# interstellar/zkvm

Measured on AMD Instinct MI355X. Metric: ZkVM tx verifications/sec (batch), higher is better.
Workload: dtype u32 limb pairs of radix-2^51 (v_mad_u64_u32)

## Files before the change

zkvm_amd/csrc/kernels.hpp:

```cpp
#pragma once
#include "curve.hpp"
#include "quad.hpp"
#include "sc_dev.hpp"

namespace zk {

constexpr uint32_t ENTRY_NEG = 1u << 31;
constexpr uint32_t ENTRY_DYN = 1u << 30;
constexpr uint32_t ENTRY_IDX = (1u << 30) - 1;
constexpr int NIELS_WORDS = 32;
constexpr int EXT_WORDS = 40;
constexpr int REDUCE_CHUNK = 64;
#ifndef ZK_REDUCE_CHUNK_BIG
#define ZK_REDUCE_CHUNK_BIG 16
#endif
constexpr int REDUCE_CHUNK_BIG = ZK_REDUCE_CHUNK_BIG;
constexpr int TABLE_WORDS = 24;
constexpr int TABLE_STRIDE = 32;

struct JobDesc {
  const uint32_t* dyn_scalars;
  const uint64_t* dyn_offsets;
  uint64_t n_dyn;
  const uint32_t* st_scalars;
  const uint32_t* st_index;
  const uint64_t* st_offsets;
  uint64_t n_static;
  uint32_t n_msm;
  int w;
  int n_windows;
  uint32_t n_buckets;
};


__device__ __forceinline__ void load_niels(ge_niels& q, const uint32_t* row) {
  const uint4* r4 = reinterpret_cast<const uint4*>(row);
  uint32_t w[32];
#pragma unroll
  for (int i = 0; i < 8; ++i) {
    uint4 v = r4[i];
    w[4 * i] = v.x; w[4 * i + 1] = v.y; w[4 * i + 2] = v.z; w[4 * i + 3] = v.w;
  }
#pragma unroll
  for (int i = 0; i < 10; ++i) { q.ypx.v[i] = w[i]; q.ymx.v[i] = w[10 + i]; q.xy2d.v[i] = w[20 + i]; }
}

__device__ __forceinline__ void store_niels(uint32_t* row, const ge_niels& q, uint32_t valid) {
  uint32_t w[32];
#pragma unroll
  for (int i = 0; i < 10; ++i) { w[i] = q.ypx.v[i]; w[10 + i] = q.ymx.v[i]; w[20 + i] = q.xy2d.v[i]; }
  w[30] = valid; w[31] = 0;
  uint4* r4 = reinterpret_cast<uint4*>(row);
#pragma unroll
  for (int i = 0; i < 8; ++i) r4[i] = make_uint4(w[4 * i], w[4 * i + 1], w[4 * i + 2], w[4 * i + 3]);
}

__device__ __forceinline__ void load_ext(ge& p, const uint32_t* row) {
  const uint4* r4 = reinterpret_cast<const uint4*>(row);
  uint32_t w[40];
#pragma unroll
  for (int i = 0; i < 10; ++i) {
    uint4 v = r4[i];
    w[4 * i] = v.x; w[4 * i + 1] = v.y; w[4 * i + 2] = v.z; w[4 * i + 3] = v.w;
  }
#pragma unroll
  for (int i = 0; i < 10; ++i) { p.X.v[i] = w[i]; p.Y.v[i] = w[10 + i]; p.Z.v[i] = w[20 + i]; p.T.v[i] = w[30 + i]; }
}

__device__ __forceinline__ void store_ext(uint32_t* row, const ge& p) {
  uint32_t w[40];
#pragma unroll
  for (int i = 0; i < 10; ++i) { w[i] = p.X.v[i]; w[10 + i] = p.Y.v[i]; w[20 + i] = p.Z.v[i]; w[30 + i] = p.T.v[i]; }
  uint4* r4 = reinterpret_cast<uint4*>(row);
#pragma unroll
  for (int i = 0; i < 10; ++i) r4[i] = make_uint4(w[4 * i], w[4 * i + 1], w[4 * i + 2], w[4 * i + 3]);
}

__device__ __forceinline__ void load_table_row(ge_niels& q, const uint32_t* row) {
  const uint4* r4 = reinterpret_cast<const uint4*>(row);
  uint32_t w[24];
#pragma unroll
  for (int i = 0; i < 6; ++i) {
    uint4 v = r4[i];
    w[4 * i] = v.x; w[4 * i + 1] = v.y; w[4 * i + 2] = v.z; w[4 * i + 3] = v.w;
  }
  fe_from_words(q.ypx, w);
  fe_from_words(q.ymx, w + 8);
  fe_from_words(q.xy2d, w + 16);
}

__device__ __forceinline__ void store_table_row(uint32_t* row, const ge_niels& q) {
  uint32_t w[24];
  fe_to_words(w, q.ypx);
  fe_to_words(w + 8, q.ymx);
  fe_to_words(w + 16, q.xy2d);
  uint4* r4 = reinterpret_cast<uint4*>(row);
#pragma unroll
  for (int i = 0; i < 6; ++i) r4[i] = make_uint4(w[4 * i], w[4 * i + 1], w[4 * i + 2], w[4 * i + 3]);
}

__device__ __forceinline__ uint32_t find_row(const uint64_t* __restrict__ offsets, uint32_t n_msm, uint64_t g) {
  uint32_t lo = 0, hi = n_msm;
  while (hi - lo > 1) {
    uint32_t mid = (lo + hi) >> 1;
    if (offsets[mid] <= g) lo = mid; else hi = mid;
  }
  return lo;
}

__global__ void __launch_bounds__(256)
k_decompress(const uint32_t* __restrict__ pts, uint32_t* __restrict__ rows, uint64_t n,
             const uint64_t* __restrict__ offsets, uint32_t n_msm, uint32_t* __restrict__ msm_fail,
             unsigned long long* __restrict__ bad_index, uint8_t* __restrict__ ok_out) {
  uint64_t i = (uint64_t)blockIdx.x * blockDim.x + threadIdx.x;
  if (i >= n) return;
  const uint4* p4 = reinterpret_cast<const uint4*>(pts + 8 * i);
  uint4 a = p4[0], b = p4[1];
  uint32_t w[8] = {a.x, a.y, a.z, a.w, b.x, b.y, b.z, b.w};
  fe x, y;
  bool ok = ristretto_decode_affine(x, y, w);
  ge_niels q;
  niels_from_affine(q, x, y);
  if (!ok) niels_identity(q);
  if (rows) store_niels(rows + NIELS_WORDS * i, q, ok ? 1u : 0u);
  if (ok_out) ok_out[i] = ok ? 1 : 0;
  if (!ok) {
    if (bad_index) atomicMin(bad_index, (unsigned long long)i);
    if (msm_fail) {
      uint32_t m = (n_msm > 1 && offsets) ? find_row(offsets, n_msm, i) : 0;
      atomicOr(&msm_fail[m], 1u);
    }
  }
}

struct DecodeRoutes {
  uint64_t n[4] = {0, 0, 0, 0};
  void note(bool split, uint64_t points) {
    n[split ? 2 : 0] += 1;
    n[split ? 3 : 1] += points;
  }
};

constexpr int DEC_WORDS = 64;

struct DecFront { fe s, u1, u2, v, w, w7; bool pre_ok; };
__device__ __forceinline__ void dec_front(DecFront& d, const uint32_t* __restrict__ pts, uint64_t i) {
  const uint4* p4 = reinterpret_cast<const uint4*>(pts + 8 * i);
  uint4 a = p4[0], b = p4[1];
  uint32_t w[8] = {a.x, a.y, a.z, a.w, b.x, b.y, b.z, b.w};
  fe ss, u2_sqr, t;
  fe_from_words(d.s, w);
  uint32_t chk[8];
  fe_to_words(chk, d.s);
  bool canonical = true;
#pragma unroll
  for (int k = 0; k < 8; ++k) canonical &= (chk[k] == w[k]);
  d.pre_ok = canonical && !(w[0] & 1);
  fe_sq(ss, d.s);
  fe_sub(d.u1, fe_one(), ss);
  fe_add(d.u2, fe_one(), ss);
  fe_carry(d.u1);
  fe_carry(d.u2);
  fe_sq(u2_sqr, d.u2);
  fe_sq(t, d.u1);
  fe_mul(t, t, fe_D());
  fe_add(t, t, u2_sqr);
  fe_sub_c(d.v, fe_zero(), t);
  fe_mul(d.w, d.v, u2_sqr);
  fe w2, w3;
  fe_sq(w2, d.w);
  fe_mul(w3, w2, d.w);
  fe_sq(d.w7, w3);
  fe_mul(d.w7, d.w7, d.w);
}

__global__ void __launch_bounds__(256)
k_decompress_pre(const uint32_t* __restrict__ pts, uint32_t* __restrict__ scratch, uint64_t n) {
  const uint64_t i = (uint64_t)blockIdx.x * blockDim.x + threadIdx.x;
  if (i >= n) return;
  DecFront d;
  dec_front(d, pts, i);
  uint32_t* col = scratch + (uint64_t)50 * n + i;
#pragma unroll
  for (int k = 0; k < 10; ++k) col[(uint64_t)k * n] = d.w7.v[k];
}

#ifndef ZK_POW_WAVES
#define ZK_POW_WAVES 3
#endif
__global__ void __launch_bounds__(256, ZK_POW_WAVES)
k_pow22523(uint32_t* __restrict__ scratch, uint64_t n) {
  const uint64_t i = (uint64_t)blockIdx.x * blockDim.x + threadIdx.x;
  if (i >= n) return;
  uint32_t* col = scratch + (uint64_t)50 * n + i;
  fe x, r;
#pragma unroll
  for (int k = 0; k < 10; ++k) x.v[k] = col[(uint64_t)k * n];
  fe_pow22523(r, x);
#pragma unroll
  for (int k = 0; k < 10; ++k) col[(uint64_t)k * n] = r.v[k];
}

__global__ void __launch_bounds__(256)
k_decompress_post(const uint32_t* __restrict__ pts, const uint32_t* __restrict__ scratch, uint32_t* __restrict__ rows, uint64_t n,
                  const uint64_t* __restrict__ offsets, uint32_t n_msm, uint32_t* __restrict__ msm_fail,
                  unsigned long long* __restrict__ bad_index) {
  const uint64_t i = (uint64_t)blockIdx.x * blockDim.x + threadIdx.x;
  if (i >= n) return;
  DecFront d;
  dec_front(d, pts, i);
  const fe s = d.s, u1 = d.u1, u2 = d.u2, v = d.v, w = d.w;
  const bool pre_ok = d.pre_ok;
  const uint32_t* col = scratch + (uint64_t)50 * n + i;
  fe pw;
#pragma unroll
  for (int k = 0; k < 10; ++k) pw.v[k] = col[(uint64_t)k * n];
  fe w3, r, t, check, r_prime, neg_r;
  fe_sq(t, w);
  fe_mul(w3, t, w);
  fe_mul(r, pw, w3);
  fe_sq(t, r);
  fe_mul(check, t, w);
  const fe one = fe_one();
  fe neg_one, neg_i;
  fe_neg(neg_one, one);
  fe_mul(neg_i, neg_one, fe_SQRT_M1());
  const bool correct_sign = fe_eq(check, one);
  const bool flipped_sign = fe_eq(check, neg_one);
  const bool flipped_sign_i = fe_eq(check, neg_i);
  fe_mul(r_prime, r, fe_SQRT_M1());
  fe_cmov(r, r_prime, flipped_sign | flipped_sign_i);
  fe_neg(neg_r, r);
  fe_cmov(r, neg_r, fe_is_negative(r));
  const bool was_square = correct_sign | flipped_sign;
  fe den_x, den_y, x, y, nx;
  fe_mul(den_x, r, u2);
  fe_mul(den_y, r, den_x);
  fe_mul(den_y, den_y, v);
  fe_mul(x, s, den_x);
  fe_add(x, x, x);
  fe_carry(x);
  fe_neg(nx, x);
  fe_cmov(x, nx, fe_is_negative(x));
  fe_mul(y, u1, den_y);
  fe_mul(t, x, y);
  const bool ok = pre_ok & was_square & !fe_is_negative(t) & !fe_is_zero(y);
  ge_niels q;
  niels_from_affine(q, x, y);
  if (!ok) niels_identity(q);
  store_niels(rows + NIELS_WORDS * i, q, ok ? 1u : 0u);
  if (!ok) {
    if (bad_index) atomicMin(bad_index, (unsigned long long)i);
    if (msm_fail) {
      uint32_t m = (n_msm > 1 && offsets) ? find_row(offsets, n_msm, i) : 0;
      atomicOr(&msm_fail[m], 1u);
    }
  }
}

template <typename F>
__device__ __forceinline__ void for_each_digit(const uint32_t* __restrict__ sc, int w, int n_windows, F f) {
  uint32_t s[8];
  const uint4* s4 = reinterpret_cast<const uint4*>(sc);
  uint4 a = s4[0], b = s4[1];
  s[0] = a.x; s[1] = a.y; s[2] = a.z; s[3] = a.w; s[4] = b.x; s[5] = b.y; s[6] = b.z; s[7] = b.w;
  const uint32_t mask = (1u << w) - 1, half = 1u << (w - 1);
  uint32_t carry = 0;
  for (int t = 0; t < n_windows; ++t) {
    const int pos = t * w;
    uint32_t bits = 0;
    if (pos < 256) {
      const int idx = pos >> 5, sh = pos & 31;
      uint32_t lo = 0, hi = 0;
#pragma unroll
      for (int k = 0; k < 8; ++k) { lo = (k == idx) ? s[k] : lo; hi = (k == idx + 1) ? s[k] : hi; }
      uint64_t two = (uint64_t)lo | ((uint64_t)hi << 32);
      bits = (uint32_t)(two >> sh) & mask;
    }
    uint32_t v = bits + carry;
    int d;
    if (v > half) { d = (int)v - (int)(mask + 1); carry = 1; }
    else { d = (int)v; carry = 0; }
    if (d != 0) f(t, d);
  }
}

__device__ __forceinline__ void term_lookup(const JobDesc& j, uint64_t g, const uint32_t*& sc, uint32_t& m,
                                            uint32_t& entry) {
  if (g < j.n_dyn) {
    sc = j.dyn_scalars + 8 * g;
    m = (j.n_msm > 1) ? find_row(j.dyn_offsets, j.n_msm, g) : 0;
    entry = ENTRY_DYN | (uint32_t)g;
  } else {
    const uint64_t k = g - j.n_dyn;
    sc = j.st_scalars + 8 * k;
    m = (j.n_msm > 1) ? find_row(j.st_offsets, j.n_msm, k) : 0;
    entry = j.st_index ? j.st_index[k] : (uint32_t)(k - (j.n_msm > 1 ? j.st_offsets[m] : 0));
  }
}

__global__ void __launch_bounds__(256)
k_digits_count(JobDesc j, uint32_t* __restrict__ hist, uint32_t* __restrict__ status) {
  uint64_t g = (uint64_t)blockIdx.x * blockDim.x + threadIdx.x;
  if (g >= j.n_dyn + j.n_static) return;
  const uint32_t* sc; uint32_t m, entry;
  term_lookup(j, g, sc, m, entry);
  if (sc[7] >> 31) atomicOr(&status[0], 2u);
  const uint64_t base = (uint64_t)m * j.n_windows;
  for_each_digit(sc, j.w, j.n_windows, [&](int t, int d) {
    const uint32_t b = (uint32_t)(d < 0 ? -d : d) - 1;
    atomicAdd(&hist[(base + t) * j.n_buckets + b], 1u);
  });
}

__global__ void __launch_bounds__(256)
k_digits_scatter(JobDesc j, uint32_t* __restrict__ cursor, uint32_t* __restrict__ entries) {
  uint64_t g = (uint64_t)blockIdx.x * blockDim.x + threadIdx.x;
  if (g >= j.n_dyn + j.n_static) return;
  const uint32_t* sc; uint32_t m, entry;
  term_lookup(j, g, sc, m, entry);
  const uint64_t base = (uint64_t)m * j.n_windows;
  for_each_digit(sc, j.w, j.n_windows, [&](int t, int d) {
    const uint32_t b = (uint32_t)(d < 0 ? -d : d) - 1;
    const uint32_t pos = atomicAdd(&cursor[(base + t) * j.n_buckets + b], 1u);
    entries[pos] = entry | (d < 0 ? ENTRY_NEG : 0u);
  });
}

constexpr int SCAN_ITEMS = 8;
constexpr int SCAN_BLOCK = 256;
constexpr int SCAN_TILE = SCAN_ITEMS * SCAN_BLOCK;

__device__ __forceinline__ uint32_t block_exclusive_scan(uint32_t v, uint32_t& total) {
  __shared__ uint32_t wave_tot[SCAN_BLOCK / 64];
  const int lane = threadIdx.x & 63, wid = threadIdx.x >> 6;
  uint32_t x = v;
#pragma unroll
  for (int o = 1; o < 64; o <<= 1) {
    uint32_t y = __shfl_up(x, o);
    if (lane >= o) x += y;
  }
  if (lane == 63) wave_tot[wid] = x;
  __syncthreads();
  uint32_t base = 0, tot = 0;
#pragma unroll
  for (int k = 0; k < SCAN_BLOCK / 64; ++k) {
    uint32_t wt = wave_tot[k];
    if (k < wid) base += wt;
    tot += wt;
  }
  __syncthreads();
  total = tot;
  return base + x - v;
}

__global__ void __launch_bounds__(SCAN_BLOCK)
k_scan_reduce(const uint32_t* __restrict__ in, uint64_t n, uint32_t* __restrict__ block_sums) {
  const uint64_t base = (uint64_t)blockIdx.x * SCAN_TILE + (uint64_t)threadIdx.x * SCAN_ITEMS;
  uint32_t s = 0;
#pragma unroll
  for (int k = 0; k < SCAN_ITEMS; ++k) if (base + k < n) s += in[base + k];
  uint32_t total;
  (void)block_exclusive_scan(s, total);
  if (threadIdx.x == 0) block_sums[blockIdx.x] = total;
}

__global__ void __launch_bounds__(SCAN_BLOCK)
k_scan_blocksums(uint32_t* __restrict__ block_sums, uint32_t n_blocks) {
  uint32_t carry = 0;
  for (uint32_t start = 0; start < n_blocks; start += SCAN_BLOCK) {
    const uint32_t i = start + threadIdx.x;
    uint32_t v = i < n_blocks ? block_sums[i] : 0;
    uint32_t total;
    uint32_t ex = block_exclusive_scan(v, total);
    if (i < n_blocks) block_sums[i] = carry + ex;
    carry += total;
  }
}

__global__ void __launch_bounds__(SCAN_BLOCK)
k_scan_apply(uint32_t* __restrict__ data, uint64_t n, const uint32_t* __restrict__ block_sums) {
  const uint64_t base = (uint64_t)blockIdx.x * SCAN_TILE + (uint64_t)threadIdx.x * SCAN_ITEMS;
  uint32_t v[SCAN_ITEMS], s = 0;
#pragma unroll
  for (int k = 0; k < SCAN_ITEMS; ++k) { v[k] = (base + k < n) ? data[base + k] : 0; s += v[k]; }
  uint32_t total;
  uint32_t ex = block_exclusive_scan(s, total) + block_sums[blockIdx.x];
#pragma unroll
  for (int k = 0; k < SCAN_ITEMS; ++k) { if (base + k < n) data[base + k] = ex; ex += v[k]; }
}

// ... 487 lines not shown
  fe_add(h, b, a);
  fe_sub(f, d, c);
  fe_add(g, d, c);
  fe_cswap(f, g, negate);
  fe_mul(r.X, e, f);
  fe_mul(r.Y, g, h);
  fe_mul(r.Z, f, g);
  fe_mul(r.T, e, h);
}

constexpr int SMALL_TBL = 8;

__device__ __forceinline__ void store_cached(uint32_t* row, const ge& p) {
  ge c4;
  fe_add_c(c4.X, p.Y, p.X);
  fe_sub_c(c4.Y, p.Y, p.X);
  fe_add_c(c4.Z, p.Z, p.Z);
  fe_mul(c4.T, p.T, fe_D2());
  store_ext(row, c4);
}

__global__ void __launch_bounds__(64)
k_small_tables(const uint32_t* __restrict__ dyn_scalars, const uint32_t* __restrict__ dyn_rows, uint64_t n,
               uint32_t* __restrict__ tbl , uint32_t* __restrict__ recoded ,
               uint32_t* __restrict__ status) {
  const uint64_t k = (uint64_t)blockIdx.x * 64 + threadIdx.x;
  if (k >= n) return;
  if (dyn_scalars) {
    const uint32_t* sc = dyn_scalars + 8 * k;
    if (sc[7] >> 31) atomicOr(&status[0], 2u);
    uint32_t carry = 0;
#pragma unroll
    for (int i = 0; i < 8; ++i) {
      const uint64_t v = (uint64_t)sc[i] + 0x88888888u + carry;
      recoded[8 * k + i] = (uint32_t)v;
      carry = (uint32_t)(v >> 32);
    }
  }
  ge_niels nq;
  load_niels(nq, dyn_rows + k * NIELS_WORDS);
  ge cur;
  ge_identity(cur);
  uint32_t* row = tbl + k * (SMALL_TBL * EXT_WORDS);
#pragma unroll 1
  for (int e = 0; e < SMALL_TBL; ++e) {
    ge_madd(cur, cur, nq, false);
    store_cached(row + e * EXT_WORDS, cur);
  }
}

__global__ void __launch_bounds__(256)
k_small_accumulate(const uint32_t* __restrict__ recoded, const uint64_t* __restrict__ dyn_offsets,
                   const uint32_t* __restrict__ tbl, uint32_t n_msm, uint32_t* __restrict__ window_sums,
                   uint32_t* __restrict__ window_nonempty) {
  extern __shared__ __attribute__((aligned(16))) uint32_t smem[];
  const uint32_t m = blockIdx.x;
  const int t = threadIdx.x & 63;
  const int part = threadIdx.x >> 6, parts = blockDim.x >> 6;
  const uint64_t k0 = dyn_offsets[m], k1 = dyn_offsets[m + 1];
  ge total;
  bool total_set = false;
#pragma unroll 1
  for (uint64_t k = k0 + part; k < k1; k += parts) {
    const uint32_t n4 = (recoded[8 * k + (t >> 3)] >> (4 * (t & 7))) & 15u;
    const int d = (t == 63 && n4 < 8u) ? (int)n4 + 8 : (int)n4 - 8;
    if (d != 0) {
      ge c4;
      load_ext(c4, tbl + (k * SMALL_TBL + (uint64_t)((d < 0 ? -d : d) - 1)) * EXT_WORDS);
      ge_cached c;
      c.YpX = c4.X; c.YmX = c4.Y; c.Z2 = c4.Z; c.T2d = c4.T;
      if (!total_set) { ge_identity(total); total_set = true; }
      ge_add_cached(total, total, c, d < 0);
    }
  }
  if (part > 0) {
    uint32_t* slot = smem + (uint32_t)(part - 1) * 41 * 64;
    slot[40 * 64 + t] = total_set ? 1u : 0u;
    if (total_set) {
#pragma unroll
      for (int q = 0; q < 10; ++q) {
        slot[q * 64 + t] = total.X.v[q]; slot[(10 + q) * 64 + t] = total.Y.v[q];
        slot[(20 + q) * 64 + t] = total.Z.v[q]; slot[(30 + q) * 64 + t] = total.T.v[q];
      }
    }
  }
  __syncthreads();
  if (part != 0) return;
#pragma unroll 1
  for (int o = 1; o < parts; ++o) {
    const uint32_t* slot = smem + (uint32_t)(o - 1) * 41 * 64;
    if (slot[40 * 64 + t]) {
      ge other;
#pragma unroll
      for (int q = 0; q < 10; ++q) {
        other.X.v[q] = slot[q * 64 + t]; other.Y.v[q] = slot[(10 + q) * 64 + t];
        other.Z.v[q] = slot[(20 + q) * 64 + t]; other.T.v[q] = slot[(30 + q) * 64 + t];
      }
      if (total_set) ge_add(total, total, other); else { total = other; total_set = true; }
    }
  }
  const uint64_t win = (uint64_t)m * 64 + t;
  window_nonempty[win] = total_set ? 1u : 0u;
  if (total_set) store_ext(window_sums + win * EXT_WORDS, total);
}

__global__ void __launch_bounds__(256)
k_msm_finish_quad(const uint32_t* __restrict__ window_sums, const uint32_t* __restrict__ window_nonempty,
                  const uint32_t* __restrict__ msm_fail, uint8_t* __restrict__ accept,
                  uint32_t* __restrict__ out_enc, uint32_t* __restrict__ out_ext, uint32_t n_msm, int w,
                  int n_windows, const uint32_t* __restrict__ sel_state, uint32_t sel_group) {
  const uint32_t g = blockIdx.x * blockDim.x + threadIdx.x;
  const int r = g & 3;
  const bool live = (g >> 2) < n_msm;
  const uint32_t m = live ? (g >> 2) : (n_msm - 1);
  if (sel_state && sel_state[m / sel_group] == 0) return;
  ge acc;
  ge_identity(acc);
  bool have = false;
  const uint64_t win0 = (uint64_t)m * n_windows;
  ge p;
  uint32_t ne = window_nonempty[win0 + n_windows - 1];
  load_ext(p, window_sums + (win0 + n_windows - 1) * EXT_WORDS);
  for (int t = n_windows - 1; t >= 0; --t) {
    ge pn;
    uint32_t nen = 0;
    if (t > 0) {
      nen = window_nonempty[win0 + t - 1];
      load_ext(pn, window_sums + (win0 + t - 1) * EXT_WORDS);
    }
    if (have) {
      for (int k = 0; k < w; ++k) quad_double(acc, r);
    }
    if (ne) {
      if (have) quad_add(acc, p, r); else { acc = p; have = true; }
    }
    if (t > 0) { p = pn; ne = nen; }
  }
  if (!live || r != 0) return;
  const bool failed = msm_fail && msm_fail[m];
  if (out_ext) {
    store_ext(out_ext + (uint64_t)m * EXT_WORDS, acc);
    if (accept) accept[m] = failed ? 0 : 1;
    return;
  }
  if (out_enc) {
    uint32_t enc[8] = {0, 0, 0, 0, 0, 0, 0, 0};
    if (have && !failed) ristretto_encode(enc, acc);
    uint4* o = reinterpret_cast<uint4*>(out_enc + 8 * (uint64_t)m);
    o[0] = make_uint4(enc[0], enc[1], enc[2], enc[3]);
    o[1] = make_uint4(enc[4], enc[5], enc[6], enc[7]);
    accept[m] = failed ? 0 : 1;
    return;
  }
  const bool ident = have ? ge_is_identity(acc) : true;
  accept[m] = (ident && !failed) ? 1 : 0;
}

__global__ void __launch_bounds__(64)
k_from_uniform(const uint32_t* __restrict__ in, uint32_t* __restrict__ out, uint64_t n) {
  const uint64_t i = (uint64_t)blockIdx.x * blockDim.x + threadIdx.x;
  if (i >= n) return;
  uint32_t w[16];
  const uint4* i4 = reinterpret_cast<const uint4*>(in + 16 * i);
#pragma unroll
  for (int k = 0; k < 4; ++k) { uint4 v = i4[k]; w[4 * k] = v.x; w[4 * k + 1] = v.y; w[4 * k + 2] = v.z; w[4 * k + 3] = v.w; }
  ge p;
  ristretto_from_uniform_words(p, w);
  uint32_t enc[8];
  ristretto_encode(enc, p);
  uint4* o = reinterpret_cast<uint4*>(out + 8 * i);
  o[0] = make_uint4(enc[0], enc[1], enc[2], enc[3]);
  o[1] = make_uint4(enc[4], enc[5], enc[6], enc[7]);
}

__global__ void __launch_bounds__(64)
k_spin(unsigned long long cycles, uint32_t* __restrict__ sink) {
  const unsigned long long t0 = clock64();
  unsigned long long spins = 0;
  while ((unsigned long long)clock64() - t0 < cycles) ++spins;
  if (sink && spins == ~0ull) *sink = 1;
}

__global__ void __launch_bounds__(256)
k_hbm_copy(const uint4* __restrict__ src, uint4* __restrict__ dst, uint64_t n_vec) {
  const uint64_t i = (uint64_t)blockIdx.x * 256 + threadIdx.x;
  if (i < n_vec) dst[i] = src[i];
}

__global__ void __launch_bounds__(256)
k_batch_init(uint32_t* __restrict__ status, uint32_t* __restrict__ msm_fail, uint32_t* __restrict__ wellformed,
             uint32_t n_msm) {
  const uint32_t i = blockIdx.x * blockDim.x + threadIdx.x;
  if (i < n_msm) {
    msm_fail[i] = 0;
    if (wellformed) wellformed[i] = 0xffffffffu;
  }
  if (i == 0) {
    status[0] = 0; status[1] = 0;
    status[2] = 0xffffffffu; status[3] = 0xffffffffu;
    status[8] = 0;
    status[9] = 0;
  }
}

__global__ void __launch_bounds__(256)
k_pack_bitmap(const uint8_t* __restrict__ accept, const uint32_t* __restrict__ wellformed ,
              uint8_t* __restrict__ bitmap, uint32_t n_msm) {
  const uint32_t byte = blockIdx.x * blockDim.x + threadIdx.x;
  if (byte >= (n_msm + 7) / 8) return;
  uint32_t v = 0;
#pragma unroll
  for (int k = 0; k < 8; ++k) {
    const uint32_t i = byte * 8 + k;
    if (i < n_msm && accept[i] && (!wellformed || wellformed[i])) v |= 1u << k;
  }
  bitmap[byte] = (uint8_t)v;
}


__global__ void __launch_bounds__(64)
k_tbl_base(const uint32_t* __restrict__ rows , uint32_t* __restrict__ base, uint32_t n_set, int w, int W) {
  const uint32_t j = blockIdx.x * blockDim.x + threadIdx.x;
  if (j >= n_set) return;
  ge_niels q;
  load_niels(q, rows + (uint64_t)j * NIELS_WORDS);
  ge p;
  ge_identity(p);
  ge_madd(p, p, q, false);
  for (int t = 0; t < W; ++t) {
    store_ext(base + ((uint64_t)t * n_set + j) * EXT_WORDS, p);
    if (t + 1 < W) {
      for (int k = 0; k < w - 1; ++k) ge_double<false>(p, p);
      ge_double<true>(p, p);
    }
  }
}

__global__ void __launch_bounds__(64)
k_tbl_multiples(const uint32_t* __restrict__ base, uint32_t* __restrict__ tmp, uint32_t* __restrict__ table,
                uint64_t n_lanes, uint32_t H) {
  const uint64_t lane = (uint64_t)blockIdx.x * blockDim.x + threadIdx.x;
  if (lane >= n_lanes) return;
  ge p, q;
  load_ext(p, base + lane * EXT_WORDS);
  q = p;
  fe prod = fe_one();
  uint32_t* mytmp = tmp + lane * (uint64_t)H * EXT_WORDS;
  for (uint32_t d = 0; d < H; ++d) {
    if (d) ge_add(q, q, p);
    fe_mul(prod, prod, q.Z);
    ge rec;
    rec.X = q.X; rec.Y = q.Y; rec.Z = q.Z; rec.T = prod;
    store_ext(mytmp + (uint64_t)d * EXT_WORDS, rec);
  }
  fe inv;
  fe_invert(inv, prod);
  uint32_t* myrows = table + lane * (uint64_t)H * TABLE_STRIDE;
  for (uint32_t d = H; d-- > 0;) {
    ge rec;
    load_ext(rec, mytmp + (uint64_t)d * EXT_WORDS);
    fe prev = fe_one();
    if (d) {
      ge r2;
      load_ext(r2, mytmp + (uint64_t)(d - 1) * EXT_WORDS);
      prev = r2.T;
    }
    fe zinv, x, y;
    fe_mul(zinv, inv, prev);
    fe_mul(inv, inv, rec.Z);
    fe_mul(x, rec.X, zinv);
    fe_mul(y, rec.Y, zinv);
    ge_niels nq;
    niels_from_affine(nq, x, y);
    store_table_row(myrows + (uint64_t)d * TABLE_STRIDE, nq);
  }
}

__global__ void __launch_bounds__(256)
k_static_digits(const uint32_t* __restrict__ st_scalars, int16_t* __restrict__ digits, uint64_t n_static, int w,
                int W, uint32_t* __restrict__ status, const uint32_t* __restrict__ row_map ,
                const uint32_t* __restrict__ n_active , uint32_t rows_per_msm, uint32_t fold_small_negatives) {
  uint64_t k = (uint64_t)blockIdx.x * blockDim.x + threadIdx.x;
  if (k >= n_static) return;
  if (row_map) {
    const uint32_t slot = (uint32_t)(k / rows_per_msm);
    if (slot >= *n_active) return;
    k = (uint64_t)row_map[slot] * rows_per_msm + k % rows_per_msm;
  }
  const uint32_t* sc = st_scalars + 8 * k;
  if (sc[7] >> 31) atomicOr(&status[0], 2u);
  for (int t = 0; t < W; ++t) digits[(uint64_t)t * n_static + k] = 0;
  if (fold_small_negatives) {
    const uint32_t l[8] = ZK_SC_L;
    uint32_t v[8];
    uint64_t br = 0;
    for (int i = 0; i < 8; ++i) { const uint64_t d = (uint64_t)l[i] - sc[i] - br; v[i] = (uint32_t)d; br = (d >> 32) & 1; }
    uint32_t high = v[0] >> 14;
    for (int i = 1; i < 8; ++i) high |= v[i];
    if (br == 0 && high == 0 && v[0] != 0 && w >= 15) { digits[k] = (int16_t)(-(int)v[0]); return; }
  }
  for_each_digit(sc, w, W, [&](int t, int d) { digits[(uint64_t)t * n_static + k] = (int16_t)d; });
}

template <bool kSkipZeros>
__global__ void __launch_bounds__(256)
k_static_accumulate(const int16_t* __restrict__ digits, const uint64_t* __restrict__ st_offsets,
                    const uint32_t* __restrict__ st_index, const uint32_t* __restrict__ table, uint32_t n_set,
                    uint32_t H, int W, int P, uint32_t n_msm, uint64_t n_static, uint32_t* __restrict__ partials,
                    const uint32_t* __restrict__ row_map ,
                    const uint32_t* __restrict__ n_active ,
                    uint32_t interleave ) {
  const uint64_t lane = (uint64_t)blockIdx.x * blockDim.x + threadIdx.x;
  if (lane >= (uint64_t)n_msm * W * P) return;
  const uint32_t part = (uint32_t)(lane % P);
  uint32_t slot = (uint32_t)((lane / P) % n_msm);
  const uint32_t t = (uint32_t)(lane / ((uint64_t)P * n_msm));
  if (n_active && slot >= *n_active) return;
  if (interleave > 1) { const uint32_t per = n_msm / interleave; slot = (slot % per) * interleave + slot / per; }
  const uint32_t tx = row_map ? row_map[slot] : slot;
  const uint64_t k0 = st_offsets[tx], k1 = st_offsets[tx + 1];
  const int16_t* dig = digits + (uint64_t)t * n_static;
  const uint64_t tbase = (uint64_t)t * n_set;
  ge acc;
  ge_identity(acc);
  auto fetch = [&](uint64_t k, ge_niels& q, bool& neg, bool& any) {
    int d = dig[k];
    d = (d == -32768) ? 32768 : d;
    any = d != 0;
    const uint32_t idx = st_index ? st_index[k] : (uint32_t)(k - k0);
    const uint32_t mag = (uint32_t)(d < 0 ? -d : d);
    if (!kSkipZeros || any) load_table_row(q, table + ((tbase + idx) * H + (mag ? mag - 1 : 0)) * TABLE_STRIDE);
    if (!any) niels_identity(q);
    neg = d < 0;
  };
  uint64_t k = k0 + part;
  ge_niels cur, nxt;
  bool cur_neg = false, nxt_neg = false, cur_any = false, nxt_any = false;
  if (k < k1) fetch(k, cur, cur_neg, cur_any);
  while (k < k1) {
    const uint64_t kn = k + P;
    if (kn < k1) fetch(kn, nxt, nxt_neg, nxt_any);
    if (!kSkipZeros || __any(cur_any)) ge_madd(acc, acc, cur, cur_neg);
    cur = nxt; cur_neg = nxt_neg; cur_any = nxt_any;
    k = kn;
  }
  store_ext(partials + (((uint64_t)slot * W + t) * P + part) * EXT_WORDS, acc);
}

__device__ inline void static_combine_slot(const uint32_t* __restrict__ partials, uint32_t n_partials, const uint32_t* __restrict__ dyn_sum,
                                           const uint8_t* __restrict__ dyn_ok, uint32_t slot, uint32_t tx, int lane,
                                           uint8_t* __restrict__ accept, uint32_t* __restrict__ out_points) {
  ge acc;
  ge_identity(acc);
  for (uint32_t c = lane; c < n_partials; c += 64) {
    ge p;
    load_ext(p, partials + ((uint64_t)slot * n_partials + c) * EXT_WORDS);
    ge_add(acc, acc, p);
  }
  if (lane == 0 && dyn_sum) {
    ge p;
    load_ext(p, dyn_sum + (uint64_t)tx * EXT_WORDS);
    ge_add(acc, acc, p);
  }
#pragma unroll 1
  for (int delta = 32; delta >= 1; delta >>= 1) {
    ge other;
    shfl_down_ge(other, acc, delta);
    if (lane < delta) ge_add(acc, acc, other);
  }
  if (lane == 0) {
    accept[tx] = (ge_is_identity(acc) && (!dyn_ok || dyn_ok[tx])) ? 1 : 0;
    if (out_points) store_ext(out_points + (uint64_t)slot * EXT_WORDS, acc);
  }
}

constexpr uint32_t COMBINE_LANES = 8;

__global__ void __launch_bounds__(64)
k_static_combine(const uint32_t* __restrict__ partials, uint32_t n_partials, const uint32_t* __restrict__ dyn_sum,
                 const uint8_t* __restrict__ dyn_ok, const uint32_t* __restrict__ row_map,
                 const uint32_t* __restrict__ n_active, uint32_t n_slots, uint8_t* __restrict__ accept,
                 uint32_t* __restrict__ out_points ) {
  const uint32_t n = n_active ? min(*n_active, n_slots) : n_slots;
  const uint32_t g = blockIdx.x * 64 + threadIdx.x, sub = g % COMBINE_LANES, first = (blockIdx.x * 64) / COMBINE_LANES;
  if (first >= n) return;
  const uint32_t mine = g / COMBINE_LANES, slot = mine < n ? mine : n - 1;
  const uint32_t tx = row_map ? row_map[slot] : slot;
  ge acc;
  ge_identity(acc);
  for (uint32_t c = sub; c < n_partials; c += COMBINE_LANES) {
    ge p;
    load_ext(p, partials + ((uint64_t)slot * n_partials + c) * EXT_WORDS);
    ge_add(acc, acc, p);
  }
  if (sub == 0 && dyn_sum) {
    ge p;
    load_ext(p, dyn_sum + (uint64_t)tx * EXT_WORDS);
    ge_add(acc, acc, p);
  }
#pragma unroll 1
  for (int delta = COMBINE_LANES / 2; delta >= 1; delta >>= 1) {
    ge other;
    shfl_down_ge(other, acc, delta);
    if (sub < (uint32_t)delta) ge_add(acc, acc, other);
  }
  if (sub == 0 && mine < n) {
    accept[tx] = (ge_is_identity(acc) && (!dyn_ok || dyn_ok[tx])) ? 1 : 0;
    if (out_points) store_ext(out_points + (uint64_t)slot * EXT_WORDS, acc);
  }
}

__device__ inline void static_row_share(ge& acc, const int16_t* __restrict__ digits, uint64_t n_static_total, uint64_t k0, uint32_t ns,
                                        const uint32_t* __restrict__ st_index, const uint32_t* __restrict__ table, uint32_t n_set,
                                        uint32_t H, int W, uint32_t tid, uint32_t n_threads) {
  ge_identity(acc);
  const uint32_t items = (uint32_t)W * ns;
  auto fetch = [&](uint32_t i, ge_niels& q, bool& neg) {
    const uint32_t t = i / ns, j = i - t * ns;
    const uint64_t k = k0 + j;
    int d = digits[(uint64_t)t * n_static_total + k];
    d = (d == -32768) ? 32768 : d;
    const uint32_t idx = st_index ? st_index[k] : j;
    const uint32_t mag = (uint32_t)(d < 0 ? -d : d);
    load_table_row(q, table + (((uint64_t)t * n_set + idx) * H + (mag ? mag - 1 : 0)) * TABLE_STRIDE);
    if (d == 0) niels_identity(q);
    neg = d < 0;
  };
  uint32_t i = tid;
  ge_niels cur, nxt;
  bool cur_neg = false, nxt_neg = false;
  if (i < items) fetch(i, cur, cur_neg);
  while (i < items) {
    const uint32_t in = i + n_threads;
    if (in < items) fetch(in, nxt, nxt_neg);
    ge_madd(acc, acc, cur, cur_neg);
    cur = nxt; cur_neg = nxt_neg;
    i = in;
  }
}

__global__ void __launch_bounds__(512)
k_recheck_fused(const int16_t* __restrict__ digits, const uint64_t* __restrict__ st_offsets, const uint32_t* __restrict__ st_index,
                const uint32_t* __restrict__ table, uint32_t n_set, uint32_t H, int W, uint64_t n_static_total,
                uint32_t* __restrict__ partials , const uint32_t* __restrict__ dyn_sum,
                const uint8_t* __restrict__ dyn_ok, const uint32_t* __restrict__ row_map, const uint32_t* __restrict__ n_active,
                uint8_t* __restrict__ accept, uint32_t* __restrict__ out_points) {
  const uint32_t slot = blockIdx.x;
  if (slot >= *n_active) return;
  const uint32_t tx = row_map[slot];
  const uint64_t k0 = st_offsets[tx];
  ge acc;
  static_row_share(acc, digits, n_static_total, k0, (uint32_t)(st_offsets[tx + 1] - k0), st_index, table, n_set, H, W, threadIdx.x, blockDim.x);
  store_ext(partials + ((uint64_t)slot * blockDim.x + threadIdx.x) * EXT_WORDS, acc);
  __threadfence_block();
  __syncthreads();
  if (threadIdx.x < 64) static_combine_slot(partials, blockDim.x, dyn_sum, dyn_ok, slot, tx, (int)threadIdx.x, accept, out_points);
}

__global__ void __launch_bounds__(64)
k_static_values(const uint32_t* __restrict__ partials, uint32_t n_partials, uint32_t* __restrict__ out_enc) {
  const uint32_t m = blockIdx.x;
  const int lane = threadIdx.x;
  ge acc;
  ge_identity(acc);
  for (uint32_t c = lane; c < n_partials; c += 64) {
    ge p;
    load_ext(p, partials + ((uint64_t)m * n_partials + c) * EXT_WORDS);
    ge_add(acc, acc, p);
  }
#pragma unroll 1
  for (int delta = 32; delta >= 1; delta >>= 1) {
    ge other;
    shfl_down_ge(other, acc, delta);
    if (lane < delta) ge_add(acc, acc, other);
  }
  if (lane == 0) {
    uint32_t enc[8];
    ristretto_encode(enc, acc);
    uint4* o = reinterpret_cast<uint4*>(out_enc + 8 * (uint64_t)m);
    o[0] = make_uint4(enc[0], enc[1], enc[2], enc[3]);
    o[1] = make_uint4(enc[4], enc[5], enc[6], enc[7]);
  }
}

constexpr uint32_t ROW_SUM_LANES = 8;
__global__ void __launch_bounds__(64)
k_static_row_sums(const uint32_t* __restrict__ partials, uint32_t n_partials, uint32_t n_rows, uint32_t* __restrict__ out_ext) {
  const uint32_t g = blockIdx.x * 64 + threadIdx.x, sub = g % ROW_SUM_LANES;
  const uint32_t row = g / ROW_SUM_LANES, m = row < n_rows ? row : n_rows - 1;
  ge acc;
  ge_identity(acc);
  for (uint32_t c = sub; c < n_partials; c += ROW_SUM_LANES) {
    ge p;
    load_ext(p, partials + ((uint64_t)m * n_partials + c) * EXT_WORDS);
    ge_add(acc, acc, p);
  }
#pragma unroll 1
  for (int delta = ROW_SUM_LANES / 2; delta >= 1; delta >>= 1) {
    ge other;
    shfl_down_ge(other, acc, delta);
    if (sub < (uint32_t)delta) ge_add(acc, acc, other);
  }
  if (sub == 0 && row < n_rows) store_ext(out_ext + (uint64_t)row * EXT_WORDS, acc);
}
__global__ void __launch_bounds__(64)
k_encode_rows(const uint32_t* __restrict__ ext, uint32_t n_rows, uint32_t* __restrict__ out_enc) {
  const uint32_t m = blockIdx.x * blockDim.x + threadIdx.x;
  if (m >= n_rows) return;
  ge p;
  load_ext(p, ext + (uint64_t)m * EXT_WORDS);
  uint32_t enc[8];
  ristretto_encode(enc, p);
  uint4* o = reinterpret_cast<uint4*>(out_enc + 8 * (uint64_t)m);
  o[0] = make_uint4(enc[0], enc[1], enc[2], enc[3]);
  o[1] = make_uint4(enc[4], enc[5], enc[6], enc[7]);
}

struct MergeSources {
  const uint4* com[16];
  const uint8_t* proofs[16];
  const uint4* r[16];
  uint32_t first[17];
  uint32_t n;
};
__global__ void __launch_bounds__(256)
k_merge_inputs(MergeSources src, uint32_t com_vec , uint32_t proof_len, uint4* __restrict__ com,
               uint8_t* __restrict__ proofs, uint4* __restrict__ r) {
  const uint32_t total = src.first[src.n];
  const uint64_t n_com = (uint64_t)total * com_vec, n_r = (uint64_t)total * 4, n_pw = ((uint64_t)total * proof_len + 3) / 4;
  const uint64_t g0 = (uint64_t)blockIdx.x * blockDim.x + threadIdx.x, stride = (uint64_t)gridDim.x * blockDim.x;
  auto source_of = [&src](uint32_t tx) { uint32_t k = 0; while (k + 1 < src.n && tx >= src.first[k + 1]) ++k; return k; };
  for (uint64_t g = g0; g < n_com; g += stride) {
    const uint32_t tx = (uint32_t)(g / com_vec), k = source_of(tx);
    com[g] = src.com[k][g - (uint64_t)src.first[k] * com_vec];
  }
  for (uint64_t g = g0; g < n_r; g += stride) {
    const uint32_t tx = (uint32_t)(g / 4), k = source_of(tx);
    if (src.r[k]) r[g] = src.r[k][g - (uint64_t)src.first[k] * 4];
  }
  const uint64_t n_bytes = (uint64_t)total * proof_len;
  for (uint64_t g = g0; g < n_pw; g += stride) {
    const uint64_t at0 = 4 * g;
    const uint32_t tx0 = (uint32_t)(at0 / proof_len), k0 = source_of(tx0);
    const uint64_t lo_b = (uint64_t)src.first[k0] * proof_len, hi_b = (uint64_t)src.first[k0 + 1] * proof_len;
    uint32_t w = 0;
    if (at0 >= lo_b + 4 && at0 + 12 <= hi_b) {
      const uint8_t* p = src.proofs[k0] + (at0 - lo_b);
      const uintptr_t a = (uintptr_t)p & ~(uintptr_t)3;
      const uint32_t sh = (uint32_t)((uintptr_t)p & 3);
      const uint32_t w0 = *reinterpret_cast<const uint32_t*>(a), w1 = *reinterpret_cast<const uint32_t*>(a + 4);
      w = __builtin_amdgcn_alignbyte(w1, w0, sh);
    } else {
      for (int b = 0; b < 4; ++b) {
        const uint64_t at = at0 + b;
        if (at >= n_bytes) break;
        const uint32_t tx = (uint32_t)(at / proof_len), k = source_of(tx);
        w |= (uint32_t)src.proofs[k][at - (uint64_t)src.first[k] * proof_len] << (8 * b);
      }
    }
    reinterpret_cast<uint32_t*>(proofs)[g] = w;
  }
}

constexpr uint32_t LOCATE_NONE = 0xffffffffu;

__device__ __forceinline__ bool tx_excluded(const uint32_t* __restrict__ msm_fail, const uint32_t* __restrict__ wellformed, uint32_t tx) {
  return (msm_fail && msm_fail[tx]) || (wellformed && !wellformed[tx]);
}

__device__ inline void ge_small_mul(ge& r, const ge& p, uint32_t k, int bits) {
  ge_identity(r);
#pragma unroll 1
  for (int bit = bits - 1; bit >= 0; --bit) {
    ge d;
    ge_double<true>(d, r);
    r = d;
    ge s;
    ge_add(s, r, p);
    if ((k >> bit) & 1) r = s;
  }
}

__device__ inline bool ge_ristretto_eq(const ge& p, const ge& q) {
  fe a, b, c, d;
  fe_mul(a, p.X, q.Y);
  fe_mul(b, p.Y, q.X);
  fe_mul(c, p.Y, q.Y);
  fe_mul(d, p.X, q.X);
  return fe_eq(a, b) | fe_eq(c, d);
}

__device__ __forceinline__ void shfl_ge(ge& out, const ge& in, int src_lane) {
#pragma unroll
  for (int i = 0; i < 10; ++i) {
    out.X.v[i] = __shfl(in.X.v[i], src_lane);
    out.Y.v[i] = __shfl(in.Y.v[i], src_lane);
    out.Z.v[i] = __shfl(in.Z.v[i], src_lane);
    out.T.v[i] = __shfl(in.T.v[i], src_lane);
  }
}

__global__ void __launch_bounds__(256)
k_group_windows(const uint32_t* __restrict__ window_sums, const uint32_t* __restrict__ window_nonempty,
                const uint32_t* __restrict__ msm_fail, const uint32_t* __restrict__ wellformed, uint32_t n_msm,
                uint32_t group, uint32_t n_windows, uint32_t* __restrict__ out_sums, uint32_t* __restrict__ out_nonempty) {
  const uint32_t g = blockIdx.x * blockDim.x + threadIdx.x;
  const uint32_t n_groups = (n_msm + group - 1) / group;
  if (g >= n_groups * n_windows) return;
  const uint32_t G = g / n_windows, t = g % n_windows;
  ge acc;
  bool have = false;
#pragma unroll 1
  for (uint32_t i = 0; i < group; ++i) {
    const uint32_t tx = G * group + i;
    if (tx >= n_msm) break;
    if (tx_excluded(msm_fail, wellformed, tx)) continue;
    const uint64_t win = (uint64_t)tx * n_windows + t;
    if (!window_nonempty[win]) continue;
    ge p;
    load_ext(p, window_sums + win * EXT_WORDS);
    if (have) ge_add(acc, acc, p); else { acc = p; have = true; }
  }
  out_nonempty[g] = have ? 1u : 0u;
  if (have) store_ext(out_sums + (uint64_t)g * EXT_WORDS, acc);
}

__device__ inline void locate_group(const uint32_t* __restrict__ partials2, uint32_t n_partials, const uint32_t* __restrict__ dyn_sum,
                                    const uint32_t* __restrict__ msm_fail, const uint32_t* __restrict__ wellformed, uint32_t n_msm,
                                    uint32_t group, uint32_t G, uint32_t f, const uint32_t* __restrict__ fail_sum,
                                    uint32_t* __restrict__ row_map, uint32_t* __restrict__ n_recheck, uint32_t* __restrict__ cand,
                                    const uint32_t* __restrict__ st_scalars, uint32_t n_static, int16_t* __restrict__ digits, int w, int W,
                                    unsigned long long* sh_queue);

template <bool kSpec>
__global__ void __launch_bounds__(256)
k_group_combine(const uint32_t* __restrict__ partials, uint32_t n_partials, const uint32_t* __restrict__ grp_dyn ,
                const uint32_t* __restrict__ dyn_sum, const uint32_t* __restrict__ msm_fail, const uint32_t* __restrict__ wellformed, uint32_t n_msm,
                uint32_t group, uint8_t* __restrict__ accept, uint32_t* __restrict__ grp_state ,
                uint32_t* __restrict__ fail_list, uint32_t* __restrict__ fail_sum , uint32_t* __restrict__ n_fail,
                const uint32_t* __restrict__ st_scalars, uint32_t n_static, uint32_t* __restrict__ loc_sc ,
                int16_t* __restrict__ loc_digits, int w, int W, uint32_t locate ,
                uint32_t* __restrict__ row_map, uint32_t* __restrict__ n_recheck, uint32_t* __restrict__ cand,
                int16_t* __restrict__ rechk_digits ) {
  __shared__ uint32_t sh_fail;
  __shared__ unsigned long long sh_queue;
  const uint32_t G = blockIdx.x;
  const int t = threadIdx.x, lane = t & 63;
  const uint32_t in_group = min(group, n_msm - G * group);
  if (t < 64) {
    ge acc;
    ge_identity(acc);
    for (uint32_t c = lane; c < n_partials; c += 64) {
      ge p;
      load_ext(p, partials + ((uint64_t)G * n_partials + c) * EXT_WORDS);
      ge_add(acc, acc, p);
    }
    if (grp_dyn) {
      if (lane == 0) {
        ge p;
        load_ext(p, grp_dyn + (uint64_t)G * EXT_WORDS);
        ge_add(acc, acc, p);
      }
    } else {
      for (uint32_t i = lane; i < group; i += 64) {
        const uint32_t tx = G * group + i;
        if (tx < n_msm && !tx_excluded(msm_fail, wellformed, tx)) {
          ge p;
          load_ext(p, dyn_sum + (uint64_t)tx * EXT_WORDS);
          ge_add(acc, acc, p);
        }
      }
    }
#pragma unroll 1
    for (int delta = 32; delta >= 1; delta >>= 1) {
      ge other;
      shfl_down_ge(other, acc, delta);
      if (lane < delta) ge_add(acc, acc, other);
    }
    const int ok = __shfl((lane == 0 && ge_is_identity(acc)) ? 1 : 0, 0);
    for (uint32_t i = lane; i < in_group; i += 64) {
      const uint32_t tx = G * group + i;
      accept[tx] = (ok && !tx_excluded(msm_fail, wellformed, tx)) ? 1 : 0;
    }
    if (lane == 0) {
      uint32_t f1 = 0;
      if (!ok) {
        const uint32_t f = atomicAdd(n_fail, 1u);
        fail_list[f] = G;
        store_ext(fail_sum + (uint64_t)f * EXT_WORDS, acc);
        f1 = f + 1;
      }
      grp_state[G] = f1;
      sh_fail = f1;
    }
    if (!ok && !locate) {
      unsigned long long lives = 0;
      for (uint32_t i0 = 0; i0 < in_group; i0 += 64) {
        const uint32_t i = i0 + lane, tx = G * group + i;
        const bool live = i < in_group && !tx_excluded(msm_fail, wellformed, tx);
        lives = __ballot(live);
        uint32_t base = 0;
        if (lane == 0) base = atomicAdd(n_recheck, (uint32_t)__popcll(lives));
        base = __shfl(base, 0);
        if (live) row_map[base + (uint32_t)__popcll(lives & ((1ull << lane) - 1))] = tx;
      }
    }
  }
  __syncthreads();
  const uint32_t f1 = sh_fail;
  if (f1 == 0) return;
  const uint32_t f = f1 - 1;
  if (!locate) { if (t == 0) cand[f] = LOCATE_NONE; return; }
  if (kSpec && locate == 2) {
    const uint32_t n_groups2 = (n_msm + group - 1) / group;
    locate_group(partials + (uint64_t)(n_groups2 + G) * n_partials * EXT_WORDS, n_partials, dyn_sum, msm_fail, wellformed, n_msm, group, G, f,
                 fail_sum, row_map, n_recheck, cand, st_scalars, n_static, rechk_digits, w, W, &sh_queue);
    return;
  }
  const uint32_t n_groups = (n_msm + group - 1) / group;
  const uint64_t stride = (uint64_t)n_groups * n_static;
  for (uint32_t j = (uint32_t)t; j < n_static; j += blockDim.x) {
    scm run = scm_zero(), sum = scm_zero();
    for (uint32_t i = in_group; i-- > 0;) {
      const uint32_t tx = G * group + i;
      if (!tx_excluded(msm_fail, wellformed, tx)) {
        const uint4* src = reinterpret_cast<const uint4*>(st_scalars + ((uint64_t)tx * n_static + j) * 8);
        const uint4 a = src[0], b = src[1];
        scm v;
        v.v[0] = a.x; v.v[1] = a.y; v.v[2] = a.z; v.v[3] = a.w; v.v[4] = b.x; v.v[5] = b.y; v.v[6] = b.z; v.v[7] = b.w;
        run = scm_add(run, v);
      }
      sum = scm_add(sum, run);
    }
    uint32_t* o = loc_sc + ((uint64_t)f * n_static + j) * 8;
    uint4* dst = reinterpret_cast<uint4*>(o);
    dst[0] = make_uint4(sum.v[0], sum.v[1], sum.v[2], sum.v[3]);
    dst[1] = make_uint4(sum.v[4], sum.v[5], sum.v[6], sum.v[7]);
    const uint64_t g = (uint64_t)f * n_static + j;
    for (int tt = 0; tt < W; ++tt) loc_digits[(uint64_t)tt * stride + g] = 0;
    for_each_digit(o, w, W, [&](int tt, int d) { loc_digits[(uint64_t)tt * stride + g] = (int16_t)d; });
  }
// ... 159 lines not shown
```

Baseline: 3.431 million.

## Software-pipeline table row loads with raw vector registers and sched barriers

Splits the table row load into an issue step that fills raw 128-bit vector registers and a separate unpack step. A shared helper pipelines the accumulation loops so the digit load runs two iterations ahead and the table row load one iteration ahead. Scheduling barriers pin the memory issue before the point-add so it can overlap with it. This is meant to hide global memory latency behind the curve arithmetic, at the cost of extra live registers that may lower occupancy.

```diff
diff --git a/zkvm_amd/csrc/kernels.hpp b/zkvm_amd/csrc/kernels.hpp
--- a/zkvm_amd/csrc/kernels.hpp
+++ b/zkvm_amd/csrc/kernels.hpp
@@ -76,17 +76,30 @@
   for (int i = 0; i < 10; ++i) r4[i] = make_uint4(w[4 * i], w[4 * i + 1], w[4 * i + 2], w[4 * i + 3]);
 }
 
-__device__ __forceinline__ void load_table_row(ge_niels& q, const uint32_t* row) {
-  const uint4* r4 = reinterpret_cast<const uint4*>(row);
+typedef uint32_t table_row_quad __attribute__((ext_vector_type(4)));
+struct table_row_raw {
+  table_row_quad v[6];
+};
+
+__device__ __forceinline__ void issue_table_row(table_row_raw& r, const uint32_t* row) {
+  const table_row_quad* r4 = reinterpret_cast<const table_row_quad*>(row);
+#pragma unroll
+  for (int i = 0; i < 6; ++i) r.v[i] = r4[i];
+}
+
+__device__ __forceinline__ void unpack_table_row(ge_niels& q, const table_row_raw& r) {
   uint32_t w[24];
 #pragma unroll
-  for (int i = 0; i < 6; ++i) {
-    uint4 v = r4[i];
-    w[4 * i] = v.x; w[4 * i + 1] = v.y; w[4 * i + 2] = v.z; w[4 * i + 3] = v.w;
-  }
+  for (int i = 0; i < 6; ++i) { w[4 * i] = r.v[i].x; w[4 * i + 1] = r.v[i].y; w[4 * i + 2] = r.v[i].z; w[4 * i + 3] = r.v[i].w; }
   fe_from_words(q.ypx, w);
   fe_from_words(q.ymx, w + 8);
   fe_from_words(q.xy2d, w + 16);
+}
+
+__device__ __forceinline__ void load_table_row(ge_niels& q, const uint32_t* row) {
+  table_row_raw r;
+  issue_table_row(r, row);
+  unpack_table_row(q, r);
 }
 
 __device__ __forceinline__ void store_table_row(uint32_t* row, const ge_niels& q) {
@@ -1180,6 +1193,48 @@
   for_each_digit(sc, w, W, [&](int t, int d) { digits[(uint64_t)t * n_static + k] = (int16_t)d; });
 }
 
+struct table_term {
+  const int16_t* digit;
+  const uint32_t* index;
+  uint32_t pos;
+  uint64_t tbase;
+};
+
+template <bool kSkipZeros, class Place>
+__device__ __forceinline__ void table_terms_sum(ge& acc, uint32_t count, const uint32_t* __restrict__ table, uint32_t H, Place place) {
+  table_row_raw raw = {};
+  ge_niels cur;
+  int16_t dig = 0;
+  uint32_t idx = 0;
+  uint64_t tbase = 0;
+  bool raw_neg = false, raw_any = false;
+  auto issue_digit = [&](uint32_t n) {
+    const table_term p = place(n);
+    dig = *p.digit;
+    idx = p.index ? *p.index : p.pos;
+    tbase = p.tbase;
+  };
+  auto issue_row = [&]() {
+    const int d = (dig == -32768) ? 32768 : dig;
+    raw_any = d != 0;
+    raw_neg = d < 0;
+    const uint32_t mag = (uint32_t)(d < 0 ? -d : d);
+    if (!kSkipZeros || raw_any) issue_table_row(raw, table + ((tbase + idx) * H + (mag ? mag - 1 : 0)) * TABLE_STRIDE);
+  };
+  if (count > 0) { issue_digit(0); issue_row(); }
+  if (count > 1) issue_digit(1);
+  for (uint32_t n = 0; n < count; ++n) {
+    unpack_table_row(cur, raw);
+    if (!raw_any) niels_identity(cur);
+    const bool cur_neg = raw_neg, cur_any = raw_any;
+    if (n + 1 < count) issue_row();
+    if (n + 2 < count) issue_digit(n + 2);
+    __builtin_amdgcn_sched_barrier(0);
+    if (!kSkipZeros || __any(cur_any)) ge_madd(acc, acc, cur, cur_neg);
+    __builtin_amdgcn_sched_barrier(0);
+  }
+}
+
 template <bool kSkipZeros>
 __global__ void __launch_bounds__(256)
 k_static_accumulate(const int16_t* __restrict__ digits, const uint64_t* __restrict__ st_offsets,
@@ -1201,27 +1256,11 @@
   const uint64_t tbase = (uint64_t)t * n_set;
   ge acc;
   ge_identity(acc);
-  auto fetch = [&](uint64_t k, ge_niels& q, bool& neg, bool& any) {
-    int d = dig[k];
-    d = (d == -32768) ? 32768 : d;
-    any = d != 0;
-    const uint32_t idx = st_index ? st_index[k] : (uint32_t)(k - k0);
-    const uint32_t mag = (uint32_t)(d < 0 ? -d : d);
-    if (!kSkipZeros || any) load_table_row(q, table + ((tbase + idx) * H + (mag ? mag - 1 : 0)) * TABLE_STRIDE);
-    if (!any) niels_identity(q);
-    neg = d < 0;
-  };
-  uint64_t k = k0 + part;
-  ge_niels cur, nxt;
-  bool cur_neg = false, nxt_neg = false, cur_any = false, nxt_any = false;
-  if (k < k1) fetch(k, cur, cur_neg, cur_any);
-  while (k < k1) {
-    const uint64_t kn = k + P;
-    if (kn < k1) fetch(kn, nxt, nxt_neg, nxt_any);
-    if (!kSkipZeros || __any(cur_any)) ge_madd(acc, acc, cur, cur_neg);
-    cur = nxt; cur_neg = nxt_neg; cur_any = nxt_any;
-    k = kn;
-  }
+  const uint32_t ns = (uint32_t)(k1 - k0), count = part < ns ? (ns - part + (uint32_t)P - 1) / (uint32_t)P : 0;
+  table_terms_sum<kSkipZeros>(acc, count, table, H, [&](uint32_t n) {
+    const uint64_t k = k0 + part + (uint64_t)n * P;
+    return table_term{dig + k, st_index ? st_index + k : nullptr, (uint32_t)(k - k0), tbase};
+  });
   store_ext(partials + (((uint64_t)slot * W + t) * P + part) * EXT_WORDS, acc);
 }
 
@@ -1293,28 +1332,12 @@
                                         uint32_t H, int W, uint32_t tid, uint32_t n_threads) {
   ge_identity(acc);
   const uint32_t items = (uint32_t)W * ns;
-  auto fetch = [&](uint32_t i, ge_niels& q, bool& neg) {
-    const uint32_t t = i / ns, j = i - t * ns;
+  const uint32_t count = tid < items ? (items - tid + n_threads - 1) / n_threads : 0;
+  table_terms_sum<false>(acc, count, table, H, [&](uint32_t n) {
+    const uint32_t i = tid + n * n_threads, t = i / ns, j = i - t * ns;
     const uint64_t k = k0 + j;
-    int d = digits[(uint64_t)t * n_static_total + k];
-    d = (d == -32768) ? 32768 : d;
-    const uint32_t idx = st_index ? st_index[k] : j;
-    const uint32_t mag = (uint32_t)(d < 0 ? -d : d);
-    load_table_row(q, table + (((uint64_t)t * n_set + idx) * H + (mag ? mag - 1 : 0)) * TABLE_STRIDE);
-    if (d == 0) niels_identity(q);
-    neg = d < 0;
-  };
-  uint32_t i = tid;
-  ge_niels cur, nxt;
-  bool cur_neg = false, nxt_neg = false;
-  if (i < items) fetch(i, cur, cur_neg);
-  while (i < items) {
-    const uint32_t in = i + n_threads;
-    if (in < items) fetch(in, nxt, nxt_neg);
-    ge_madd(acc, acc, cur, cur_neg);
-    cur = nxt; cur_neg = nxt_neg;
-    i = in;
-  }
+    return table_term{digits + (uint64_t)t * n_static_total + k, st_index ? st_index + k : nullptr, j, (uint64_t)t * n_set};
+  });
 }
 
 __global__ void __launch_bounds__(512)
```

Result: no change. 3.417 million (-0.4%).
